# AlphaMistral/Mistral-Water

Measured on AMD Instinct MI355X. Metric: ocean grid-points/sec (full spectrum→IFFT→disp→Jacobian), 1024² grid, 1/2/4/8 GPUs, higher is better.
Workload: dtype f32

## Files before the change

### mistral-water_amd/csrc/ocean_renderer_device.h

```cpp
#pragma once
#include <hip/hip_runtime.h>

#include <mutex>
#include <utility>
#include <vector>

#include "../../include/mistral_water.h"
#include "mw_host.h"
#include "ocean_renderer_kernels.h"
#include "mw_switches.h"

namespace mw {

struct OrTex {
    float* height = nullptr;
    cf* disp = nullptr;
    float *disp_g = nullptr, *normal = nullptr, *white = nullptr;
    float *height_g = nullptr, *disp_a = nullptr;
    OrTex at(size_t texels) const {
        auto mv = [texels](auto* p, size_t per) { return p ? p + per * texels : p; };
        return OrTex{mv(height, 1), mv(disp, 1), mv(disp_g, 1), mv(normal, 3), mv(white, 1), mv(height_g, 1), mv(disp_a, 1)};
    }
    OrTex real_only() const { OrTex t = *this; t.height_g = t.disp_a = nullptr; return t; }
};
// ... 64 lines not shown
#ifndef MW_OR_PACKED_MAX_M
#define MW_OR_PACKED_MAX_M 4096
#endif
#ifndef MW_OR_PACKED
#define MW_OR_PACKED 1
#endif

template <int N, int P>
__global__ __launch_bounds__((OrP1Geom<N, P>::NTHREADS)) void k_or_pass1_packed(OrP1Args A) {
    extern __shared__ __attribute__((aligned(16))) unsigned char smem[];
    using G = OrP1Geom<N, P>;
    cf* lds = reinterpret_cast<cf*>(smem);
    constexpr int T = FftGeom<N, P>::T;
    const int tid = threadIdx.x, jb = blockIdx.x;
    const int f0 = gridDim.y == 1 ? 0 : (int)blockIdx.y, f1 = gridDim.y == 1 ? 2 : f0 + 1;
    {
        const size_t toff = (size_t)blockIdx.z * N * N;
        A.initT += toff; A.PQT += toff; A.phase_in += toff; A.phase_out += toff; A.E += 2 * toff;
    }
    const int w = tid / T, u = tid % T;
    TwStage<N, P, G::NTHREADS, false> tws;
    tws.load(A.TW, tid);
    const Twiddles tw = TwGeom<N, P>::view(A.TW, lds);
    cf* set0 = lds + G::TW_LDS;
    cf h[P], hh[P], x[P];
#pragma unroll
    for (int q = 0; q < P; q++) h[q] = hh[q] = mk(0.f, 0.f);
    if (gridDim.y == 1) or_p1_animate_packed<N, P, MW_OR_P1_CHUNK>(A, jb, tid, true, true, true, h, hh);
    else or_p1_animate_packed<N, P, MW_OR_P1_LONE_CHUNK>(A, jb, tid, f0 == 0, f0 == 0, f0 == 1, h, hh);
    tws.store(lds, tid);
    for (int f = f0; f < f1; f++) {
        or_p1_build_packed<N, P>(A, jb, tid, f, h, hh, x);
        if (f != f0) __syncthreads();
        stage0_store<N, P, -1>(x, u, set0 + w * G::BUFSTRIDE);
        __syncthreads();
#pragma unroll
        for (int s = 1; s < FftGeom<N, P>::S; s++) {
            load_slots<N, P>(x, u, set0 + w * G::BUFSTRIDE, s - 1);
            __syncthreads();
            stage_store<N, P, -1, false>(x, u, set0 + w * G::BUFSTRIDE, tw, s);
            __syncthreads();
        }
        or_p1_finish<N, P>(A, tw, jb, tid, f, x, set0);
    }
}

template <int N, int P>
__global__ __launch_bounds__((OrP1Geom<N, P>::NTHREADS)) void k_or_pass1(OrP1Args A) {
    extern __shared__ __attribute__((aligned(16))) unsigned char smem[];
    using G = OrP1Geom<N, P>;
    cf* lds = reinterpret_cast<cf*>(smem);
    constexpr int T = FftGeom<N, P>::T;
    const int tid = threadIdx.x, jb = blockIdx.x;
    const int f0 = gridDim.y == 1 ? 0 : (int)blockIdx.y, f1 = gridDim.y == 1 ? 3 : f0 + 1;
    {
        const size_t toff = (size_t)blockIdx.z * N * N;
        A.initT += toff; A.phase_in += toff; A.phase_out += toff; A.E += 3 * toff;
    }
    const int w = tid / T, u = tid % T;
    TwStage<N, P, G::NTHREADS, false> tws;
    tws.load(A.TW, tid);
    const Twiddles tw = TwGeom<N, P>::view(A.TW, lds);
    cf* set0 = lds + G::TW_LDS;
    cf h[P], x[P];
    if (gridDim.y == 1) or_p1_animate<N, P, MW_OR_P1_CHUNK>(A, jb, tid, f0 == 0, h);
    else or_p1_animate<N, P, 1>(A, jb, tid, f0 == 0, h);
    tws.store(lds, tid);
    for (int f = f0; f < f1; f++) {
        or_p1_build<N, P>(A, jb, tid, f, h, x);
        if (f != f0) __syncthreads();
        stage0_store<N, P, -1>(x, u, set0 + w * G::BUFSTRIDE);
        __syncthreads();
#pragma unroll
        for (int s = 1; s < FftGeom<N, P>::S; s++) {
            load_slots<N, P>(x, u, set0 + w * G::BUFSTRIDE, s - 1);
            __syncthreads();
            stage_store<N, P, -1, false>(x, u, set0 + w * G::BUFSTRIDE, tw, s);
            __syncthreads();
        }
        or_p1_finish<N, P>(A, tw, jb, tid, f, x, set0);
    }
}

template <int N, int P, bool KEEP, bool PACKED = false>
__global__ __launch_bounds__((OrP1Geom<N, P>::NTHREADS)) void k_or_pass1_steps(OrP1StepsArgs S) {
    constexpr int NF = PACKED ? 2 : 3;
    extern __shared__ __attribute__((aligned(16))) unsigned char smem[];
    using G = OrP1Geom<N, P>;
    cf* lds = reinterpret_cast<cf*>(smem);
    constexpr int T = FftGeom<N, P>::T;
    const int tid = threadIdx.x, jb = blockIdx.x;
    const int k0 = (int)blockIdx.z * S.group, k1 = (k0 + S.group < S.nframes) ? k0 + S.group : S.nframes;
    OrP1Args A = S.a;
    const int w = tid / T, u = tid % T;
    TwStage<N, P, G::NTHREADS, false> tws;
    tws.load(A.TW, tid);
    const Twiddles tw = TwGeom<N, P>::view(A.TW, lds);
    cf* set0 = lds + G::TW_LDS;
    float om[P], ph[P];
    f4 v[P], vn;
    const int fsel = PACKED ? (int)blockIdx.y : 0;
    or_p1_steps_begin<N, P>(A, jb, tid, om, ph);
    float gain[PACKED ? P : 1];
    if constexpr (PACKED) {
        if (KEEP) or_p1_steps_coeff<N, P>(A, jb, tid, fsel, v, vn);
        or_p1_steps_gain<N, P>(A, jb, tid, fsel, gain);
    }
    else { if (KEEP) or_p1_steps_spectrum<N, P>(A, jb, tid, v); }
    tws.store(lds, tid);
    for (int k = 0; k < k0; k++) or_p1_steps_advance<P>(om, ph, S.dt[k]);
    A.E += (size_t)NF * N * N * k0;
    for (int k = k0; k < k1; k++) {
        cf h[PACKED ? 1 : P], x[P];
        or_p1_steps_advance<P>(om, ph, S.dt[k]);
        if constexpr (PACKED) {
            if (!KEEP) or_p1_steps_coeff<N, P>(A, jb, tid, fsel, v, vn);
        } else {
            if (!KEEP) or_p1_steps_spectrum<N, P>(A, jb, tid, v);
            or_p1_steps_animate<P>(v, ph, h);
        }
        for (int f = PACKED ? fsel : 0; f < (PACKED ? fsel + 1 : 3); f++) {
            if constexpr (PACKED) or_p1_steps_build_split<N, P>(tid, f, gain, v, vn, ph, x);
            else or_p1_build<N, P>(A, jb, tid, f, h, x);
            if ((!PACKED && f != 0) || k != k0) __syncthreads();
            stage0_store<N, P, -1>(x, u, set0 + w * G::BUFSTRIDE);
            __syncthreads();
#pragma unroll
            for (int s = 1; s < FftGeom<N, P>::S; s++) {
                load_slots<N, P>(x, u, set0 + w * G::BUFSTRIDE, s - 1);
                __syncthreads();
                stage_store<N, P, -1, false>(x, u, set0 + w * G::BUFSTRIDE, tw, s);
                __syncthreads();
            }
            or_p1_finish<N, P>(A, tw, jb, tid, f, x, set0);
        }
        A.E += (size_t)NF * N * N;
    }
    if (k1 == S.nframes && fsel == 0) or_p1_steps_store_phase<N, P>(A, jb, tid, ph);
}

__global__ __launch_bounds__(256) void k_or_copy_frame(size_t MM, const float* h, const cf* d, const float* dg, const float* n, const float* w,
                                                       const float* hg, const float* da, float* oh, cf* od, float* odg, float* on, float* ow,
                                                       float* ohg, float* oda) {
    const size_t i = (size_t)blockIdx.x * blockDim.x + threadIdx.x, q = MM / 4;
    auto cp = [i](const void* src, void* dst) { reinterpret_cast<f4*>(dst)[i] = reinterpret_cast<const f4*>(src)[i]; };
    if (i < 3 * q) cp(n, on);
    if (i < 2 * q) cp(d, od);
    if (i < q) {
        cp(h, oh); cp(dg, odg); cp(w, ow);
        if (hg) { cp(hg, ohg); cp(da, oda); }
    }
}

__device__ __forceinline__ unsigned or_xcd_band(unsigned b, unsigned nb) { return (nb % 8 == 0) ? (b % 8) * (nb / 8) + b / 8 : b; }
template <int N, int P>
__global__ __launch_bounds__((OrP2Geom<N, P>::NTHREADS)) void k_or_pass2(OrP2Args A) {
    extern __shared__ __attribute__((aligned(16))) unsigned char smem[];
    using G = OrP2Geom<N, P>;
    cf* lds = reinterpret_cast<cf*>(smem);
    constexpr int T = FftGeom<N, P>::T;
    const int tid = threadIdx.x, ab = blockIdx.x;
    {
        const size_t toff = (size_t)blockIdx.z * N * N;
        A.E += 3 * toff; A.height += toff; A.disp += toff; A.disp_g += toff;
        if (A.height_g) A.height_g += toff;
        if (A.disp_a) A.disp_a += toff;
    }
    TwStage<N, P, G::NTHREADS, false> tws;
    tws.load(A.TW, tid);
    const Twiddles tw = TwGeom<N, P>::view(A.TW, lds);
    cf* set0 = lds + G::TW_LDS;
    cf x[P];
    float dx[P];
    const int k0 = blockIdx.y == 0 ? 0 : 2, k1 = blockIdx.y == 0 ? 2 : 3;
    for (int k = k0; k < k1; k++) {
        const int f = or_p2_field(k);
        if (k != k0) __syncthreads();
        or_p2_load<N, P>(A, ab, tid, f, x, set0);
        if (k == k0) tws.store(lds, tid);
        __syncthreads();
#pragma unroll
        for (int s = 1; s < FftGeom<N, P>::S; s++) {
            const int um = XLay<N, P>::EXACT ? tid % FftGeom<N, P>::T : tid >> 2, rm = XLay<N, P>::EXACT ? tid / FftGeom<N, P>::T : tid & 3;
            load_slots<N, P>(x, um, set0 + rm * G::BUFSTRIDE, s - 1);
            __syncthreads();
            stage_store<N, P, -1, false>(x, um, set0 + rm * G::BUFSTRIDE, tw, s);
            __syncthreads();
        }
        or_p2_finish<N, P>(A, tw, ab, tid, f, x, dx, set0);
    }
}

template <int N, int P>
__global__ __launch_bounds__((OrP2Geom<N, P>::NTHREADS)) void k_or_pass2_packed(OrP2Args A) {
    extern __shared__ __attribute__((aligned(16))) unsigned char smem[];
    using G = OrP2Geom<N, P>;
    cf* lds = reinterpret_cast<cf*>(smem);
    const int tid = threadIdx.x, ab = blockIdx.x;
    {
        const size_t toff = (size_t)blockIdx.z * N * N;
        A.E += 2 * toff; A.height += toff; A.disp += toff; A.disp_g += toff;
    }
    TwStage<N, P, G::NTHREADS, false> tws;
    tws.load(A.TW, tid);
    const Twiddles tw = TwGeom<N, P>::view(A.TW, lds);
    cf* set0 = lds + G::TW_LDS;
    cf x[P];
    float dx[P];
    const bool split = gridDim.y == 2;
    const int k0 = split ? (int)blockIdx.y : 0, k1 = split ? k0 + 1 : 2;
    for (int k = k0; k < k1; k++) {
        if (k != k0) __syncthreads();
        or_p2_load<N, P>(A, ab, tid, k, x, set0);
        if (k == k0) tws.store(lds, tid);
        __syncthreads();
#pragma unroll
        for (int s = 1; s < FftGeom<N, P>::S; s++) {
            const int um = XLay<N, P>::EXACT ? tid % FftGeom<N, P>::T : tid >> 2, rm = XLay<N, P>::EXACT ? tid / FftGeom<N, P>::T : tid & 3;
            load_slots<N, P>(x, um, set0 + rm * G::BUFSTRIDE, s - 1);
            __syncthreads();
            stage_store<N, P, -1, false>(x, um, set0 + rm * G::BUFSTRIDE, tw, s);
// ... 152 lines not shown
    return A;
}
template <int N>
static hipError_t or_launch_passes(OrState& s, float dt, bool imag, hipStream_t st, hipEvent_t* ev = nullptr) {
    constexpr int P = Plan<N>::P;
    static AttrOnce attr1, attr2;
    hipError_t e = attr1.set(reinterpret_cast<const void*>(&k_or_pass1<N, P>), OrP1Geom<N, P>::LDS_BYTES);
    if (e == hipSuccess) e = attr2.set(reinterpret_cast<const void*>(&k_or_pass2<N, P>), OrP2Geom<N, P>::LDS_BYTES);
    if (e != hipSuccess) return e;
    const OrP1Args A1 = or_p1_args(s, s.initT, s.PQT, s.phaseT2, s.E, dt, or_call_is_big(s));
    const OrP2Args A2 = or_p2_args(s, s.E, imag ? s.out : s.out.real_only());
    constexpr int NT1 = OrP1Geom<N, P>::NTHREADS, LB1 = OrP1Geom<N, P>::LDS_BYTES;
    constexpr int NT2 = OrP2Geom<N, P>::NTHREADS, LB2 = OrP2Geom<N, P>::LDS_BYTES;
    const bool packed = or_use_packed(s, imag), all_fields = or_all_fields(s);
    if constexpr (N < MW_OR_PACKED_MAX_M) if (packed) {
        static AttrOnce attr1p, attr2p;
        e = attr1p.set(reinterpret_cast<const void*>(&k_or_pass1_packed<N, P>), LB1);
        if (e == hipSuccess) e = attr2p.set(reinterpret_cast<const void*>(&k_or_pass2_packed<N, P>), LB2);
        if (e != hipSuccess) return e;
        if (ev) hipEventRecord(ev[0], st);
        k_or_pass1_packed<N, P><<<dim3(N / 4, all_fields ? 1 : 2, s.tiles), dim3(NT1), LB1, st>>>(A1);
        if (ev) hipEventRecord(ev[1], st);
        std::swap(s.phaseT, s.phaseT2);
        k_or_pass2_packed<N, P><<<dim3(N / 4, all_fields ? 1 : 2, s.tiles), dim3(NT2), LB2, st>>>(A2);
        if (ev) hipEventRecord(ev[2], st);
        return hipGetLastError();
    }
    if (ev) hipEventRecord(ev[0], st);
    k_or_pass1<N, P><<<dim3(N / 4, all_fields ? 1 : 3, s.tiles), dim3(NT1), LB1, st>>>(A1);
    if (ev) hipEventRecord(ev[1], st);
    std::swap(s.phaseT, s.phaseT2);
    k_or_pass2<N, P><<<dim3(N / 4, 2, s.tiles), dim3(NT2), LB2, st>>>(A2);
    if (ev) hipEventRecord(ev[2], st);
    return hipGetLastError();
}

static inline mw_status or_generate(OrState& s, float delta_time, bool imag, float* d_height, float* d_disp, float* d_normal, float* d_white,
                                    hipStream_t st, hipEvent_t* ev = nullptr) {
    const float dt = delta_time * s.mult;
    const mw_status r = imag ? or_imag_planes(s) : MW_OK;
    if (r != MW_OK) return r;
    hipError_t e = hipSuccess;
    MW_FOR_SIZE(s.M, return fail(MW_EINVAL, "OceanRenderer: unsupported texture size"), e = or_launch_passes<NN>(s, dt, imag, st, ev));
    if (e != hipSuccess) return fail(MW_EDEVICE, std::string("OceanRenderer pass launch: ") + hipGetErrorString(e));
    const size_t MM = (size_t)s.M * s.M, TM = MM * (size_t)s.tiles;
    const unsigned nb = or_nw_blocks(MM);
    const OrTex& o = s.out;
    if (or_call_is_big(s)) k_or_normal_white<true><<<dim3(nb, s.tiles), dim3(256), 0, st>>>(s.c, o.height, o.disp, o.disp_g, o.normal, o.white);
    else k_or_normal_white<false><<<dim3(nb, s.tiles), dim3(256), 0, st>>>(s.c, o.height, o.disp, o.disp_g, o.normal, o.white);
    if (hipGetLastError() != hipSuccess) return fail(MW_EDEVICE, "OceanRenderer normal/white launch failed");
    if (ev) hipEventRecord(ev[3], st);
    s.have_frame = true;
    hipError_t ce = hipSuccess;
    if (d_height && ce == hipSuccess) ce = hipMemcpyAsync(d_height, o.height, TM * 4, hipMemcpyDeviceToDevice, st);
    if (d_disp && ce == hipSuccess) ce = hipMemcpyAsync(d_disp, o.disp, TM * 8, hipMemcpyDeviceToDevice, st);
    if (d_normal && ce == hipSuccess) ce = hipMemcpyAsync(d_normal, o.normal, TM * 12, hipMemcpyDeviceToDevice, st);
    if (d_white && ce == hipSuccess) ce = hipMemcpyAsync(d_white, o.white, TM * 4, hipMemcpyDeviceToDevice, st);
    if (ce != hipSuccess) return fail(MW_EDEVICE, std::string("OceanRenderer result copy: ") + hipGetErrorString(ce));
    if (ev) hipEventRecord(ev[4], st);
    return MW_OK;
}

static inline mw_status or_frames_reserve(OrState& s, int n, const bool (&need)[4], bool imag) {
    if (n > s.frames_cap) {
        or_release(s, OR_B_FRAMES);
        s.frames_cap = 0; s.frames_last = 0;
    }
    const size_t cap = (size_t)(s.frames_cap ? s.frames_cap : n);
    const unsigned when = OR_B_FR | (need[0] ? OR_B_FR_HEIGHT : 0u) | (need[1] ? OR_B_FR_DISP : 0u) | (need[2] ? OR_B_FR_NORMAL : 0u) |
                          (need[3] ? OR_B_FR_WHITE : 0u) | (imag ? OR_B_FR_IMAG : 0u);
    if (!or_alloc(s, when, 0, cap)) {
        (void)hipGetLastError();
        return fail(MW_ENOMEM, "OceanRenderer: hipMalloc of the frame buffers failed");
    }
    s.frames_cap = (int)cap;
    return MW_OK;
}
#ifndef MW_OR_FRAME_GROUPS
#define MW_OR_FRAME_GROUPS 4
#endif
#ifndef MW_OR_FRAME_GROUPS_PACKED
#define MW_OR_FRAME_GROUPS_PACKED 2
#endif
#ifndef MW_OR_STEPS_CHUNK
#define MW_OR_STEPS_CHUNK 8
#endif
static inline int or_steps_chunk(int M) {
    const long long c = (long long)MW_OR_STEPS_CHUNK * 1024 * 1024 / ((long long)M * M);
    return c < 1 ? 1 : (c > MW_OR_MAX_FRAMES ? MW_OR_MAX_FRAMES : (int)c);
}
static inline int or_steps_chunks(int M, int n) { const int c = or_steps_chunk(M); return (n + c - 1) / c; }
#ifndef MW_OR_STEPS_MAX_N
#define MW_OR_STEPS_MAX_N 2048
#endif
template <int N, bool PACKED>
static hipError_t or_launch_steps(OrState& s, const float* dt, int n, const OrTex& f, hipStream_t st, hipEvent_t* ev = nullptr) {
    constexpr int P = Plan<N>::P, NF = PACKED ? 2 : 3;
    constexpr bool KEEP = P <= 8;
    static AttrOnce attr1, attr2;
    {
        hipError_t e;
        if constexpr (PACKED) e = attr2.set(reinterpret_cast<const void*>(&k_or_pass2_packed<N, P>), OrP2Geom<N, P>::LDS_BYTES);
        else e = attr2.set(reinterpret_cast<const void*>(&k_or_pass2<N, P>), OrP2Geom<N, P>::LDS_BYTES);
        if (e != hipSuccess) return e;
    }
    constexpr int NT1 = OrP1Geom<N, P>::NTHREADS, LB1 = OrP1Geom<N, P>::LDS_BYTES;
    if (ev) hipEventRecord(ev[0], st);
    constexpr int NT2 = OrP2Geom<N, P>::NTHREADS, LB2 = OrP2Geom<N, P>::LDS_BYTES;
    const size_t MM = (size_t)N * N;
    const int chunk = or_steps_chunk(N);
    auto rest = [&](int c0, int cn, int j) {
        const OrTex c = f.at(MM * (size_t)c0);
        const OrP2Args B2 = or_p2_args(s, s.fr_E + NF * MM * (size_t)c0, c);
        if constexpr (PACKED) k_or_pass2_packed<N, P><<<dim3(N / 4, 1, cn), dim3(NT2), LB2, st>>>(B2);
        else k_or_pass2<N, P><<<dim3(N / 4, 2, cn), dim3(NT2), LB2, st>>>(B2);
        if (ev) hipEventRecord(ev[2 + 3 * j], st);
        k_or_normal_white<true><<<dim3(or_nw_blocks(MM), cn), dim3(256), 0, st>>>(s.c, c.height, c.disp, c.disp_g, c.normal, c.white);
        if (ev) hipEventRecord(ev[3 + 3 * j], st);
    };
    if constexpr (N <= MW_OR_STEPS_MAX_N) {
        hipError_t e = attr1.set(reinterpret_cast<const void*>(&k_or_pass1_steps<N, P, KEEP, PACKED>), LB1);
        if (e != hipSuccess) return e;
        OrP1StepsArgs S;
        S.a = or_p1_args(s, s.initT, s.PQT, s.phaseT2, s.fr_E, 0.f, true);
        for (int k = 0; k < MW_OR_MAX_FRAMES; k++) S.dt[k] = k < n ? dt[k] : 0.f;
        S.nframes = n;
        int groups = PACKED ? MW_OR_FRAME_GROUPS_PACKED : MW_OR_FRAME_GROUPS;
        if (groups > n) groups = n;
        S.group = (n + groups - 1) / groups;
        groups = (n + S.group - 1) / S.group;
        k_or_pass1_steps<N, P, KEEP, PACKED><<<dim3(N / 4, PACKED ? 2 : 1, groups), dim3(NT1), LB1, st>>>(S);
        for (int c0 = 0, j = 0; c0 < n; c0 += chunk, j++) {
            if (ev) hipEventRecord(ev[1 + 3 * j], st);
            rest(c0, (n - c0 < chunk) ? n - c0 : chunk, j);
        }
        std::swap(s.phaseT, s.phaseT2);
    } else {
        hipError_t e;
        if constexpr (PACKED) e = attr1.set(reinterpret_cast<const void*>(&k_or_pass1_packed<N, P>), LB1);
        else e = attr1.set(reinterpret_cast<const void*>(&k_or_pass1<N, P>), LB1);
        if (e != hipSuccess) return e;
        for (int c0 = 0, j = 0; c0 < n; c0 += chunk, j++) {
            const int cn = (n - c0 < chunk) ? n - c0 : chunk;
            for (int k = c0; k < c0 + cn; k++) {
                const OrP1Args A1 = or_p1_args(s, s.initT, s.PQT, s.phaseT2, s.fr_E + (size_t)NF * N * N * k, dt[k], true);
                if constexpr (PACKED) k_or_pass1_packed<N, P><<<dim3(N / 4, 1, 1), dim3(NT1), LB1, st>>>(A1);
                else k_or_pass1<N, P><<<dim3(N / 4, 1, 1), dim3(NT1), LB1, st>>>(A1);
                std::swap(s.phaseT, s.phaseT2);
            }
            if (ev) hipEventRecord(ev[1 + 3 * j], st);
            rest(c0, cn, j);
        }
    }
    return hipGetLastError();
}
static inline mw_status or_generate_steps(OrState& s, const float* delta_time, int n, bool imag, float* d_height, float* d_disp, float* d_normal,
                                          float* d_white, hipStream_t st, hipEvent_t* ev = nullptr) {
    if (s.tiles != 1) return fail(MW_ESTATE, "generate_texture_steps: a batched handle (mw_ocean_create_batch) advances one frame per call");
    if (n < 1 || n > MW_OR_MAX_FRAMES) return fail(MW_EINVAL, "generate_texture_steps: nframes out of range");
    const size_t MM = (size_t)s.M * s.M;
    mw_status r = imag ? or_imag_planes(s) : MW_OK;
    if (r != MW_OK) return r;
    const bool need[4] = {!d_height, !d_disp, !d_normal, !d_white};
    if ((r = or_frames_reserve(s, n, need, imag)) != MW_OK) return r;
    float dt[MW_OR_MAX_FRAMES];
    for (int k = 0; k < n; k++) dt[k] = delta_time[k] * s.mult;
    OrTex f = imag ? s.fr : s.fr.real_only();
    if (d_height) f.height = d_height;
    if (d_disp) f.disp = reinterpret_cast<cf*>(d_disp);
    if (d_normal) f.normal = d_normal;
    if (d_white) f.white = d_white;
    hipError_t e = hipSuccess;
    const bool packed = or_use_packed(s, imag);
    MW_FOR_SIZE(s.M, return fail(MW_EINVAL, "OceanRenderer: unsupported texture size"),
                e = packed ? or_launch_steps<NN, (NN < MW_OR_PACKED_MAX_M)>(s, dt, n, f, st, ev) : or_launch_steps<NN, false>(s, dt, n, f, st, ev));
    if (e != hipSuccess) return fail(MW_EDEVICE, std::string("OceanRenderer steps launch: ") + hipGetErrorString(e));
    const OrTex l = f.at((size_t)(n - 1) * MM), &o = s.out;
    k_or_copy_frame<<<dim3((unsigned)((3 * MM / 4 + 255) / 256)), dim3(256), 0, st>>>(MM, l.height, l.disp, l.disp_g, l.normal, l.white, l.height_g, l.disp_a,
                                                                                     o.height, o.disp, o.disp_g, o.normal, o.white, o.height_g, o.disp_a);
    if (hipGetLastError() != hipSuccess) return fail(MW_EDEVICE, "OceanRenderer normal/white launch failed");
    if (ev) hipEventRecord(ev[1 + 3 * or_steps_chunks(s.M, n)], st);
    s.have_frame = true;
    return MW_OK;
}

static inline mw_status or_frames(OrState& s, float choppiness, const float* delta_time, int n, bool rgba, void* const (&d)[4], hipStream_t st,
                                  hipEvent_t* ev = nullptr) {
    s.c.choppiness = choppiness;
    float* const p[4] = {rgba ? nullptr : (float*)d[0], rgba ? nullptr : (float*)d[1], rgba ? nullptr : (float*)d[2], rgba ? nullptr : (float*)d[3]};
    const mw_status r = n == 1 ? or_generate(s, delta_time[0], rgba, p[0], p[1], p[2], p[3], st, ev)
                               : or_generate_steps(s, delta_time, n, rgba, p[0], p[1], p[2], p[3], st, ev);
    if (r != MW_OK || !rgba) return r;
    const size_t MM = (size_t)s.M * s.M;
    const OrTex& t = n == 1 ? s.out : s.fr;
    k_or_pack_rgba<<<dim3((unsigned)((MM + 255) / 256), n == 1 ? s.tiles : n), dim3(256), 0, st>>>(s.M, t.height, t.height_g, t.disp, t.disp_g, t.disp_a, t.normal,
                                                                                              t.white, (f4*)d[0], (f4*)d[1], (f4*)d[2], (f4*)d[3]);
    if (hipGetLastError() != hipSuccess) return fail(MW_EDEVICE, "k_or_pack_rgba launch failed");
    return MW_OK;
}

struct OrAdvanceArgs {
    float dt[MW_OR_MAX_FRAMES];
    int n;
};
__global__ __launch_bounds__(256) void k_or_advance(size_t MM, const float* omT, float* phase, OrAdvanceArgs A) {
    const size_t i = (size_t)blockIdx.x * blockDim.x + threadIdx.x;
    if (i >= MM) return;
    const float om = omT[i];
    float ph = phase[i + (size_t)blockIdx.y * MM];
    for (int k = 0; k < A.n; k++) ph = or_phase_step(om, ph, A.dt[k]);
    phase[i + (size_t)blockIdx.y * MM] = ph;
}
static inline mw_status or_advance_phase(OrState& s, const float* delta_time, int n, hipStream_t st) {
    const size_t MM = (size_t)s.M * s.M;
// ... 23 lines not shown
```

### mistral-water_amd/csrc/ocean_renderer_kernels.h

```cpp
#pragma once
#include "fftmesh_kernels.h"

namespace mw {

struct OrConsts {
    int M;
    float length, gravity, choppiness;
    float normal_length;
};

MW_HD float or_wave(int M, float length, int p) {
    const float n = (float)((p < M / 2) ? p : p - M);
    return sdiv(smul(smul(2.0f, MW_PI_F), n), length);
}
MW_HD float or_phillips(int M, float length, float wind_x, float wind_y, float amp, float gravity, float kx, float kz) {
    float klen = sqrtf(kx * kx + kz * kz);
    float klen2 = klen * klen, klen4 = klen2 * klen2;
    if (klen < MW_EPS_F) return 0.f;
    float wlen = sqrtf(wind_x * wind_x + wind_y * wind_y);
    float kDotW = (kx / klen) * (wind_x / wlen) + (kz / klen) * (wind_y / wlen);
    float l = wlen * wlen / gravity, l2 = l * l;
    float damping = 0.01f, L2 = l2 * damping * damping;
    return amp * expf(-1.f / (klen2 * l2)) / klen4 * (kDotW * kDotW) * expf(-klen2 * L2);
}
// ... 17 lines not shown
    }
    f4 v;
    v.x = o[0]; v.y = o[1]; v.z = o[2]; v.w = -o[3];
    initT[(size_t)px * M + py] = v;
    if (phaseT) phaseT[(size_t)px * M + py] = 0.f;
}
MW_HD float or_omega(const OrConsts& c, int px, int py) {
    const float kx = or_wave(c.M, c.length, px), kz = or_wave(c.M, c.length, py);
    const float wlen = ssqrt(sadd(smul(kx, kx), smul(kz, kz)));
    const float q = sdiv(sdiv(smul(wlen, wlen), 370.f), 370.f);
    const float inner = smul(smul(c.gravity, wlen), sadd(1.f, q));
    return ssqrt(inner);
}
MW_HD float or_phase_step(float omega, float old_phase, float dt) {
    const float x = sadd(old_phase, smul(omega, dt)), twopi = smul(2.0f, MW_PI_F);
    if (x >= 0.f && x < twopi) return x;
    if (x >= twopi && x < sadd(twopi, twopi)) return ssub(x, twopi);
    return fmodf(x, twopi);
}
MW_HD float or_phase_advance(const OrConsts& c, int px, int py, float old_phase, float dt) {
    return or_phase_step(or_omega(c, px, py), old_phase, dt);
}

struct OrP1Args {
    const f4* PQT;
    const f4* initT;
    const float* omT;
    const float* phase_in;
    float* phase_out;
    const cf* TW;
    cf* E;
    OrConsts c;
    float dt;
    int stream_E;
};
template <int N, int P>
struct OrP1Geom {
    static constexpr int T = FftGeom<N, P>::T;
    static constexpr int NTHREADS = 4 * T;
    static constexpr int BUFSTRIDE = FftGeom<N, P>::LBUF + (XLay<N, P>::EXACT ? XLay<N, P>::PAD_RD4 : 4);
    static constexpr int TW_LDS = (TwGeom<N, P>::LDS_CF + 1) & ~1;
    static constexpr int LDS_BYTES = (TW_LDS + 4 * BUFSTRIDE) * (int)sizeof(cf);
};
#ifndef MW_OR_P1_CHUNK
#define MW_OR_P1_CHUNK 8
#endif
template <int N, int P, int CH_>
MW_HD void or_p1_animate(const OrP1Args& A, int jb, int tid, bool write_phase, cf (&h)[P]) {
    constexpr int T = FftGeom<N, P>::T;
    const int w = wave_uniform<(T % 64) == 0>(tid / T), u = tid % T, px = 4 * jb + w;
    const size_t col = (size_t)px * N;
    const float* const c_om = A.omT + col;
    const float* const c_pi = A.phase_in + col;
    float* const c_po = A.phase_out + col;
    const f4* const c_in = A.initT + col;
    const unsigned uo = (unsigned)u;
    constexpr int CH = P < CH_ ? P : CH_;
#pragma unroll
    for (int q0 = 0; q0 < P; q0 += CH) {
        float om[CH], pi[CH];
        f4 v[CH];
#pragma unroll
        for (int k = 0; k < CH; k++) {
            om[k] = (c_om + T * (q0 + k))[uo];
            pi[k] = (c_pi + T * (q0 + k))[uo];
            v[k] = (c_in + T * (q0 + k))[uo];
        }
#pragma unroll
        for (int k = 0; k < CH; k++) {
            const float ph = or_phase_step(om[k], pi[k], A.dt);
            if (write_phase) (c_po + T * (q0 + k))[uo] = ph;
            float s, c;
            mw_sincos(ph, &s, &c);
            h[q0 + k] = animate(v[k].x, v[k].y, v[k].z, v[k].w, c, s);
        }
    }
}
#define MW_OR_MAX_FRAMES 32
struct OrP1StepsArgs {
    OrP1Args a;
    float dt[MW_OR_MAX_FRAMES];
    int nframes, group;
};
template <int N, int P>
MW_HD void or_p1_steps_begin(const OrP1Args& A, int jb, int tid, float (&om)[P], float (&ph)[P]) {
    constexpr int T = FftGeom<N, P>::T;
    const int w = wave_uniform<(T % 64) == 0>(tid / T), u = tid % T, px = 4 * jb + w;
    const size_t col = (size_t)px * N;
    const float* const c_om = A.omT + col;
    const float* const c_pi = A.phase_in + col;
    const unsigned uo = (unsigned)u;
#pragma unroll
    for (int q = 0; q < P; q++) {
        om[q] = (c_om + T * q)[uo];
        ph[q] = (c_pi + T * q)[uo];
    }
}
template <int N, int P>
MW_HD void or_p1_steps_spectrum(const OrP1Args& A, int jb, int tid, f4 (&v)[P]) {
    constexpr int T = FftGeom<N, P>::T;
    const int w = wave_uniform<(T % 64) == 0>(tid / T), u = tid % T, px = 4 * jb + w;
    const f4* const c_in = A.initT + (size_t)px * N;
    const unsigned uo = (unsigned)u;
#pragma unroll
    for (int q = 0; q < P; q++) v[q] = (c_in + T * q)[uo];
}
template <int P>
MW_HD void or_p1_steps_advance(const float (&om)[P], float (&ph)[P], float dt) {
#pragma unroll
    for (int q = 0; q < P; q++) ph[q] = or_phase_step(om[q], ph[q], dt);
}
template <int P>
MW_HD void or_p1_steps_animate(const f4 (&v)[P], const float (&ph)[P], cf (&h)[P]) {
#pragma unroll
    for (int q = 0; q < P; q++) {
        float s, c;
        mw_sincos(ph[q], &s, &c);
        h[q] = animate(v[q].x, v[q].y, v[q].z, v[q].w, c, s);
    }
}
template <int N, int P>
MW_HD void or_p1_steps_store_phase(const OrP1Args& A, int jb, int tid, const float (&ph)[P]) {
    constexpr int T = FftGeom<N, P>::T;
    const int w = wave_uniform<(T % 64) == 0>(tid / T), u = tid % T, px = 4 * jb + w;
    float* const c_po = A.phase_out + (size_t)px * N;
    const unsigned uo = (unsigned)u;
#pragma unroll
    for (int q = 0; q < P; q++) (c_po + T * q)[uo] = ph[q];
}

MW_HD float or_gain(float kc, float kx, float kz, float chop) {
    const float wl = fmaxf(0.0001f, sqrtf(__builtin_fmaf(kx, kx, smul(kz, kz))));
    return smul(sdiv(kc, wl), chop);
}
template <int N, int P>
MW_HD void or_p1_build(const OrP1Args& A, int jb, int tid, int f, const cf (&h)[P], cf (&x)[P]) {
    constexpr int T = FftGeom<N, P>::T;
    const int w = tid / T, u = tid % T, px = 4 * jb + w;
    const float kx = or_wave(N, A.c.length, px);
#pragma unroll
    for (int q = 0; q < P; q++) {
        if (f == 0) { x[q] = h[q]; continue; }
        const float kz = or_wave(N, A.c.length, u + T * q);
        const float g = or_gain((f == 1) ? kx : kz, kx, kz, A.c.choppiness);
        x[q] = mk(smul(h[q].y, g), smul(-h[q].x, g));
    }
}
MW_HD void or_prep_element(int M, int px, int py, const f4* initT, f4* PQT) {
    const int mx = (M - px) % M, my = (M - py) % M;
    const f4 a = initT[(size_t)px * M + py], b = initT[(size_t)mx * M + my];
    f4 o;
    o.x = smul(0.5f, sadd(a.x, b.z)); o.y = smul(0.5f, ssub(a.y, b.w));
    o.z = smul(0.5f, sadd(a.z, b.x)); o.w = smul(0.5f, ssub(a.w, b.y));
    PQT[(size_t)px * M + py] = o;
}
template <int N, int P>
MW_HD void or_p1_build_packed(const OrP1Args& A, int jb, int tid, int f, const cf (&h)[P], const cf (&hh)[P], cf (&x)[P]) {
    constexpr int T = FftGeom<N, P>::T;
    const int w = tid / T, u = tid % T, px = 4 * jb + w;
    const float kx = or_wave(N, A.c.length, px);
#pragma unroll
    for (int q = 0; q < P; q++) {
        const int py = u + T * q;
        const float kz = or_wave(N, A.c.length, py);
        const float g = or_gain((f == 0) ? kx : kz, kx, kz, A.c.choppiness);
        if (f == 0) { x[q] = mk(smul(h[q].y, g), smul(-h[q].x, g)); continue; }
        const bool nyq = (py == N / 2);
        const float tx = nyq ? ssub(h[q].x, hh[q].x) : hh[q].x, ty = nyq ? ssub(h[q].y, hh[q].y) : hh[q].y;
        x[q] = mk(sadd(hh[q].x, smul(g, tx)), sadd(hh[q].y, smul(g, ty)));
    }
}
template <int N, int P, int CH_>
MW_HD void or_p1_animate_packed(const OrP1Args& A, int jb, int tid, bool write_phase, bool want_h, bool want_hh, cf (&h)[P], cf (&hh)[P]) {
    constexpr int T = FftGeom<N, P>::T;
    const int w = wave_uniform<(T % 64) == 0>(tid / T), u = tid % T, px = 4 * jb + w;
    const size_t col = (size_t)px * N;
    const float* const c_om = A.omT + col;
    const float* const c_pi = A.phase_in + col;
    float* const c_po = A.phase_out + col;
    const f4* const c_in = A.initT + col;
    const f4* const c_pq = A.PQT + col;
    const unsigned uo = (unsigned)u;
    constexpr int CH = P < CH_ ? P : CH_;
#pragma unroll
    for (int q0 = 0; q0 < P; q0 += CH) {
        float om[CH], pi[CH];
        f4 v[CH], pq[CH];
#pragma unroll
        for (int k = 0; k < CH; k++) {
            om[k] = (c_om + T * (q0 + k))[uo];
            pi[k] = (c_pi + T * (q0 + k))[uo];
            if (want_h || (q0 + k) == P / 2) v[k] = (c_in + T * (q0 + k))[uo];
            if (want_hh) pq[k] = (c_pq + T * (q0 + k))[uo];
        }
#pragma unroll
        for (int k = 0; k < CH; k++) {
            const float ph = or_phase_step(om[k], pi[k], A.dt);
            if (write_phase) (c_po + T * (q0 + k))[uo] = ph;
            float s, c;
            mw_sincos(ph, &s, &c);
            if (want_h || (q0 + k) == P / 2) h[q0 + k] = animate(v[k].x, v[k].y, v[k].z, v[k].w, c, s);
            if (want_hh) hh[q0 + k] = animate(pq[k].x, pq[k].y, pq[k].z, pq[k].w, c, s);
        }
    }
}
template <int N, int P>
MW_HD void or_p1_steps_coeff(const OrP1Args& A, int jb, int tid, int f, f4 (&c)[P], f4& vn) {
    constexpr int T = FftGeom<N, P>::T;
    const int w = wave_uniform<(T % 64) == 0>(tid / T), u = tid % T, px = 4 * jb + w;
    const f4* const c_c = (f == 0 ? A.initT : A.PQT) + (size_t)px * N;
    const unsigned uo = (unsigned)u;
#pragma unroll
    for (int q = 0; q < P; q++) c[q] = (c_c + T * q)[uo];
    vn = (A.initT + (size_t)px * N + T * (P / 2))[uo];
}
template <int N, int P>
MW_HD void or_p1_steps_gain(const OrP1Args& A, int jb, int tid, int f, float (&g)[P]) {
    constexpr int T = FftGeom<N, P>::T;
    const int w = tid / T, u = tid % T, px = 4 * jb + w;
    const float kx = or_wave(N, A.c.length, px);
#pragma unroll
    for (int q = 0; q < P; q++) {
        const float kz = or_wave(N, A.c.length, u + T * q);
        g[q] = or_gain((f == 0) ? kx : kz, kx, kz, A.c.choppiness);
    }
}
template <int N, int P>
MW_HD void or_p1_steps_build_split(int tid, int f, const float (&g_)[P], const f4 (&c)[P], const f4& vn, const float (&ph)[P], cf (&x)[P]) {
    constexpr int T = FftGeom<N, P>::T;
    const int u = tid % T;
#pragma unroll
    for (int q = 0; q < P; q++) {
        float sn, cs;
        mw_sincos(ph[q], &sn, &cs);
        const cf a = animate(c[q].x, c[q].y, c[q].z, c[q].w, cs, sn);
        const int py = u + T * q;
        const float g = g_[q];
        if (f == 0) { x[q] = mk(smul(a.y, g), smul(-a.x, g)); continue; }
        float tx = a.x, ty = a.y;
        if (q == P / 2) {
            const cf hn = animate(vn.x, vn.y, vn.z, vn.w, cs, sn);
            const bool nyq = (py == N / 2);
            tx = nyq ? ssub(hn.x, a.x) : a.x;
            ty = nyq ? ssub(hn.y, a.y) : a.y;
        }
        x[q] = mk(sadd(a.x, smul(g, tx)), sadd(a.y, smul(g, ty)));
    }
}

template <int N, int P>
MW_HD void or_p1_finish(const OrP1Args& A, const Twiddles& tw, int jb, int tid, int f, cf (&x)[P], const cf* lds) {
    constexpr int T = FftGeom<N, P>::T;
    const int w2 = tid & 3, u2 = tid >> 2;
    load_last<N, P>(x, u2, lds + w2 * OrP1Geom<N, P>::BUFSTRIDE);
    final_stage<N, P, -1>(x, u2, tw.TF);
    cf* Ef = A.E + (size_t)f * N * N + (size_t)jb * N * 4;
    const unsigned to = (unsigned)tid;
    if (A.stream_E) {
#pragma unroll
        for (int q = 0; q < P; q++) mw_store_stream<true>(&(Ef + (size_t)4 * T * q)[to], x[q]);
    } else {
#pragma unroll
        for (int q = 0; q < P; q++) (Ef + (size_t)4 * T * q)[to] = x[q];
    }
}

struct OrP2Args {
    const cf* E;
    const cf* TW;
    float* height;
    cf* disp;
    float* disp_g;
    float* height_g;
    float* disp_a;
    OrConsts c;
};
template <int N, int P>
struct OrP2Geom {
    static constexpr int T = FftGeom<N, P>::T;
    static constexpr int R2 = 4;
    static constexpr int NTHREADS = R2 * T;
    static constexpr int BUFSTRIDE = FftGeom<N, P>::LBUF + (XLay<N, P>::EXACT ? XLay<N, P>::PAD_WR4 : 4);
    static constexpr int TW_LDS = (TwGeom<N, P>::LDS_CF + 1) & ~1;
    static constexpr int LDS_BYTES = (TW_LDS + R2 * BUFSTRIDE) * (int)sizeof(cf);
};
MW_HD int or_p2_field(int k) { return k == 0 ? 1 : (k == 1 ? 2 : 0); }
template <int N, int P>
MW_HD void or_p2_load(const OrP2Args& A, int ab, int tid, int f, cf (&x)[P], cf* lds) {
    constexpr int T = FftGeom<N, P>::T;
    const int r1 = tid & 3, u1 = tid >> 2, row = ab * 4 + r1;
    const cf* Ef = A.E + (size_t)f * N * N;
#pragma unroll
    for (int q = 0; q < P; q++) {
        const int j = u1 + T * q;
        x[q] = Ef[((size_t)(j >> 2) * N + row) * 4 + (j & 3)];
    }
    stage0_store<N, P, -1>(x, u1, lds + r1 * OrP2Geom<N, P>::BUFSTRIDE);
}
template <int N, int P>
MW_HD void or_p2_finish(const OrP2Args& A, const Twiddles& tw, int ab, int tid, int f, cf (&x)[P], float (&dx)[P],
                        const cf* lds) {
    constexpr int T = FftGeom<N, P>::T;
    const int g = wave_uniform<(T % 64) == 0>(tid / T), u = tid % T, a = ab * 4 + g;
    load_last<N, P>(x, u, lds + g * OrP2Geom<N, P>::BUFSTRIDE);
    final_stage<N, P, -1>(x, u, tw.TF);
    const size_t rowoff = (size_t)a * N;
    float* const r_dg = A.disp_g + rowoff;
    cf* const r_d = A.disp + rowoff;
    float* const r_da = A.disp_a ? A.disp_a + rowoff : nullptr;
    float* const r_h = A.height + rowoff;
    float* const r_hg = A.height_g ? A.height_g + rowoff : nullptr;
    const unsigned uo = (unsigned)u;
#pragma unroll
    for (int q = 0; q < P; q++) {
        if (f == 1) { dx[q] = x[q].x; (r_dg + T * q)[uo] = x[q].y; }
        else if (f == 2) { (r_d + T * q)[uo] = mk(dx[q], x[q].x); if (r_da) (r_da + T * q)[uo] = x[q].y; }
        else if (f == 3) { (r_d + T * q)[uo] = mk(dx[q], x[q].y); (r_h + T * q)[uo] = x[q].x; }
        else if (f == 4) { (reinterpret_cast<float*>(r_d) + 2 * T * q)[2 * uo] = x[q].x; (r_dg + T * q)[uo] = x[q].y; }
        else if (f == 5) { (reinterpret_cast<float*>(r_d) + 2 * T * q)[2 * uo + 1] = x[q].y; (r_h + T * q)[uo] = x[q].x; }
        else { (r_h + T * q)[uo] = x[q].x; if (r_hg) (r_hg + T * q)[uo] = x[q].y; }
    }
}

MW_HD int or_clamp(int v, int hi) { return v < 0 ? 0 : (v > hi ? hi : v); }
MW_HD void or_normal_math(float ts, float cx, float cy, float cz, float rx, float rh, float rz, float lx, float lh, float lz, float tx,
                          float th, float tz, float bx, float bh, float bz, float (&n)[3]) {
    const float r0 = ts + rx - cx, r1 = rh - cy, r2 = rz - cz;
    const float l0 = -ts + lx - cx, l1 = lh - cy, l2 = lz - cz;
    const float t0 = tx - cx, t1 = th - cy, t2 = -ts + tz - cz;
    const float b0 = bx - cx, b1 = bh - cy, b2 = ts + bz - cz;
    float nx = (r1 * t2 - r2 * t1) + (t1 * l2 - t2 * l1) + (l1 * b2 - l2 * b1) + (b1 * r2 - b2 * r1);
// ... 135 lines not shown
```

Measured before the change: 82.56 billion.

## Fuse the two packed field workgroups into one and share sincos through LDS

Adds a DUO variant of the pass-1 steps kernel. It merges the two packed-field workgroups into a single double-width workgroup. Each half advances phases and computes sincos for only half of the slots, then exchanges the results through a shared LDS area. This removes the duplicated phase loads, phase advance and sincos work that both field workgroups used to repeat. The trade-offs are a larger workgroup, more LDS per block, fewer blocks (frame groups default to 1 for this path), and an extra barrier per frame, all of which could lower occupancy and parallelism.

```diff
diff --git a/mistral-water_amd/csrc/ocean_renderer_device.h b/mistral-water_amd/csrc/ocean_renderer_device.h
--- a/mistral-water_amd/csrc/ocean_renderer_device.h
+++ b/mistral-water_amd/csrc/ocean_renderer_device.h
@@ -170,47 +170,61 @@
     }
 }
 
-template <int N, int P, bool KEEP, bool PACKED = false>
-__global__ __launch_bounds__((OrP1Geom<N, P>::NTHREADS)) void k_or_pass1_steps(OrP1StepsArgs S) {
+template <int N, int P, bool KEEP, bool PACKED = false, bool DUO = false>
+__global__ __launch_bounds__(((DUO ? 2 : 1) * OrP1Geom<N, P>::NTHREADS)) void k_or_pass1_steps(OrP1StepsArgs S) {
+    static_assert(!DUO || (PACKED && KEEP && OrP1Duo<N, P>::value), "the two-field workgroup is a form of the packed plan with the coefficients kept");
     constexpr int NF = PACKED ? 2 : 3;
     extern __shared__ __attribute__((aligned(16))) unsigned char smem[];
     using G = OrP1Geom<N, P>;
     cf* lds = reinterpret_cast<cf*>(smem);
-    constexpr int T = FftGeom<N, P>::T;
-    const int tid = threadIdx.x, jb = blockIdx.x;
+    constexpr int T = FftGeom<N, P>::T, NT = G::NTHREADS;
+    constexpr int PC = DUO ? P / 2 : P;
+    const int half = DUO ? wave_uniform<(NT % 64) == 0>((int)threadIdx.x / NT) : 0;
+    const int tid = DUO ? (int)threadIdx.x - half * NT : (int)threadIdx.x, jb = blockIdx.x;
     const int k0 = (int)blockIdx.z * S.group, k1 = (k0 + S.group < S.nframes) ? k0 + S.group : S.nframes;
     OrP1Args A = S.a;
     const int w = tid / T, u = tid % T;
-    TwStage<N, P, G::NTHREADS, false> tws;
-    tws.load(A.TW, tid);
+    TwStage<N, P, (DUO ? 2 : 1) * NT, false> tws;
+    tws.load(A.TW, threadIdx.x);
     const Twiddles tw = TwGeom<N, P>::view(A.TW, lds);
-    cf* set0 = lds + G::TW_LDS;
-    float om[P], ph[P];
+    const int fsel = DUO ? half : (PACKED ? (int)blockIdx.y : 0);
+    cf* set0 = lds + G::TW_LDS + (DUO ? half * 4 * G::BUFSTRIDE : 0);
+    const int q0 = DUO ? half * PC : 0;
+    float om[PC], ph[PC];
     f4 v[P], vn;
-    const int fsel = PACKED ? (int)blockIdx.y : 0;
-    or_p1_steps_begin<N, P>(A, jb, tid, om, ph);
+    or_p1_steps_begin<N, P, PC>(A, jb, tid, q0, om, ph);
     float gain[PACKED ? P : 1];
     if constexpr (PACKED) {
         if (KEEP) or_p1_steps_coeff<N, P>(A, jb, tid, fsel, v, vn);
         or_p1_steps_gain<N, P>(A, jb, tid, fsel, gain);
     }
     else { if (KEEP) or_p1_steps_spectrum<N, P>(A, jb, tid, v); }
-    tws.store(lds, tid);
-    for (int k = 0; k < k0; k++) or_p1_steps_advance<P>(om, ph, S.dt[k]);
+    tws.store(lds, threadIdx.x);
+    for (int k = 0; k < k0; k++) or_p1_steps_advance<PC>(om, ph, S.dt[k]);
     A.E += (size_t)NF * N * N * k0;
     for (int k = k0; k < k1; k++) {
-        cf h[PACKED ? 1 : P], x[P];
-        or_p1_steps_advance<P>(om, ph, S.dt[k]);
-        if constexpr (PACKED) {
+        cf h[PACKED ? 1 : P], x[P], sc[DUO ? P : 1];
+        or_p1_steps_advance<PC>(om, ph, S.dt[k]);
+        if constexpr (DUO) {
+            cf* xs = lds + OrP1Duo<N, P>::XS;
+            cf own[PC];
+            or_p1_steps_sincos<PC>(ph, own);
+#pragma unroll
+            for (int q = 0; q < PC; q++) xs[(q0 + q) * NT + tid] = own[q];
+            __syncthreads();
+#pragma unroll
+            for (int q = 0; q < P; q++) sc[q] = xs[q * NT + tid];
+        } else if constexpr (PACKED) {
             if (!KEEP) or_p1_steps_coeff<N, P>(A, jb, tid, fsel, v, vn);
         } else {
             if (!KEEP) or_p1_steps_spectrum<N, P>(A, jb, tid, v);
             or_p1_steps_animate<P>(v, ph, h);
         }
         for (int f = PACKED ? fsel : 0; f < (PACKED ? fsel + 1 : 3); f++) {
-            if constexpr (PACKED) or_p1_steps_build_split<N, P>(tid, f, gain, v, vn, ph, x);
+            if constexpr (DUO) or_p1_steps_build_field<N, P>(tid, f, gain, v, vn, sc, x);
+            else if constexpr (PACKED) or_p1_steps_build_split<N, P>(tid, f, gain, v, vn, ph, x);
             else or_p1_build<N, P>(A, jb, tid, f, h, x);
-            if ((!PACKED && f != 0) || k != k0) __syncthreads();
+            if (!DUO && ((!PACKED && f != 0) || k != k0)) __syncthreads();
             stage0_store<N, P, -1>(x, u, set0 + w * G::BUFSTRIDE);
             __syncthreads();
 #pragma unroll
@@ -224,7 +238,7 @@
         }
         A.E += (size_t)NF * N * N;
     }
-    if (k1 == S.nframes && fsel == 0) or_p1_steps_store_phase<N, P>(A, jb, tid, ph);
+    if (k1 == S.nframes && (DUO || fsel == 0)) or_p1_steps_store_phase<N, P, PC>(A, jb, tid, q0, ph);
 }
 
 __global__ __launch_bounds__(256) void k_or_copy_frame(size_t MM, const float* h, const cf* d, const float* dg, const float* n, const float* w,
@@ -543,6 +557,9 @@
 #ifndef MW_OR_FRAME_GROUPS_PACKED
 #define MW_OR_FRAME_GROUPS_PACKED 2
 #endif
+#ifndef MW_OR_FRAME_GROUPS_DUO
+#define MW_OR_FRAME_GROUPS_DUO 1
+#endif
 #ifndef MW_OR_STEPS_CHUNK
 #define MW_OR_STEPS_CHUNK 8
 #endif
@@ -580,17 +597,19 @@
         if (ev) hipEventRecord(ev[3 + 3 * j], st);
     };
     if constexpr (N <= MW_OR_STEPS_MAX_N) {
-        hipError_t e = attr1.set(reinterpret_cast<const void*>(&k_or_pass1_steps<N, P, KEEP, PACKED>), LB1);
+        constexpr bool DUO = PACKED && KEEP && OrP1Duo<N, P>::value;
+        constexpr int NTS = DUO ? OrP1Duo<N, P>::NTHREADS : NT1, LBS = DUO ? OrP1Duo<N, P>::LDS_BYTES : LB1;
+        hipError_t e = attr1.set(reinterpret_cast<const void*>(&k_or_pass1_steps<N, P, KEEP, PACKED, DUO>), LBS);
         if (e != hipSuccess) return e;
         OrP1StepsArgs S;
         S.a = or_p1_args(s, s.initT, s.PQT, s.phaseT2, s.fr_E, 0.f, true);
         for (int k = 0; k < MW_OR_MAX_FRAMES; k++) S.dt[k] = k < n ? dt[k] : 0.f;
         S.nframes = n;
-        int groups = PACKED ? MW_OR_FRAME_GROUPS_PACKED : MW_OR_FRAME_GROUPS;
+        int groups = DUO ? MW_OR_FRAME_GROUPS_DUO : (PACKED ? MW_OR_FRAME_GROUPS_PACKED : MW_OR_FRAME_GROUPS);
         if (groups > n) groups = n;
         S.group = (n + groups - 1) / groups;
         groups = (n + S.group - 1) / S.group;
-        k_or_pass1_steps<N, P, KEEP, PACKED><<<dim3(N / 4, PACKED ? 2 : 1, groups), dim3(NT1), LB1, st>>>(S);
+        k_or_pass1_steps<N, P, KEEP, PACKED, DUO><<<dim3(N / 4, (PACKED && !DUO) ? 2 : 1, groups), dim3(NTS), LBS, st>>>(S);
         for (int c0 = 0, j = 0; c0 < n; c0 += chunk, j++) {
             if (ev) hipEventRecord(ev[1 + 3 * j], st);
             rest(c0, (n - c0 < chunk) ? n - c0 : chunk, j);
diff --git a/mistral-water_amd/csrc/ocean_renderer_kernels.h b/mistral-water_amd/csrc/ocean_renderer_kernels.h
--- a/mistral-water_amd/csrc/ocean_renderer_kernels.h
+++ b/mistral-water_amd/csrc/ocean_renderer_kernels.h
@@ -123,16 +123,16 @@
     float dt[MW_OR_MAX_FRAMES];
     int nframes, group;
 };
-template <int N, int P>
-MW_HD void or_p1_steps_begin(const OrP1Args& A, int jb, int tid, float (&om)[P], float (&ph)[P]) {
+template <int N, int P, int PC>
+MW_HD void or_p1_steps_begin(const OrP1Args& A, int jb, int tid, int q0, float (&om)[PC], float (&ph)[PC]) {
     constexpr int T = FftGeom<N, P>::T;
     const int w = wave_uniform<(T % 64) == 0>(tid / T), u = tid % T, px = 4 * jb + w;
     const size_t col = (size_t)px * N;
-    const float* const c_om = A.omT + col;
-    const float* const c_pi = A.phase_in + col;
-    const unsigned uo = (unsigned)u;
-#pragma unroll
-    for (int q = 0; q < P; q++) {
+    const float* const c_om = A.omT + col + T * q0;
+    const float* const c_pi = A.phase_in + col + T * q0;
+    const unsigned uo = (unsigned)u;
+#pragma unroll
+    for (int q = 0; q < PC; q++) {
         om[q] = (c_om + T * q)[uo];
         ph[q] = (c_pi + T * q)[uo];
     }
@@ -146,10 +146,10 @@
 #pragma unroll
     for (int q = 0; q < P; q++) v[q] = (c_in + T * q)[uo];
 }
-template <int P>
-MW_HD void or_p1_steps_advance(const float (&om)[P], float (&ph)[P], float dt) {
-#pragma unroll
-    for (int q = 0; q < P; q++) ph[q] = or_phase_step(om[q], ph[q], dt);
+template <int PC>
+MW_HD void or_p1_steps_advance(const float (&om)[PC], float (&ph)[PC], float dt) {
+#pragma unroll
+    for (int q = 0; q < PC; q++) ph[q] = or_phase_step(om[q], ph[q], dt);
 }
 template <int P>
 MW_HD void or_p1_steps_animate(const f4 (&v)[P], const float (&ph)[P], cf (&h)[P]) {
@@ -160,14 +160,14 @@
         h[q] = animate(v[q].x, v[q].y, v[q].z, v[q].w, c, s);
     }
 }
-template <int N, int P>
-MW_HD void or_p1_steps_store_phase(const OrP1Args& A, int jb, int tid, const float (&ph)[P]) {
+template <int N, int P, int PC>
+MW_HD void or_p1_steps_store_phase(const OrP1Args& A, int jb, int tid, int q0, const float (&ph)[PC]) {
     constexpr int T = FftGeom<N, P>::T;
     const int w = wave_uniform<(T % 64) == 0>(tid / T), u = tid % T, px = 4 * jb + w;
-    float* const c_po = A.phase_out + (size_t)px * N;
-    const unsigned uo = (unsigned)u;
-#pragma unroll
-    for (int q = 0; q < P; q++) (c_po + T * q)[uo] = ph[q];
+    float* const c_po = A.phase_out + (size_t)px * N + T * q0;
+    const unsigned uo = (unsigned)u;
+#pragma unroll
+    for (int q = 0; q < PC; q++) (c_po + T * q)[uo] = ph[q];
 }
 
 MW_HD float or_gain(float kc, float kx, float kz, float chop) {
@@ -266,28 +266,56 @@
         g[q] = or_gain((f == 0) ? kx : kz, kx, kz, A.c.choppiness);
     }
 }
-template <int N, int P>
-MW_HD void or_p1_steps_build_split(int tid, int f, const float (&g_)[P], const f4 (&c)[P], const f4& vn, const float (&ph)[P], cf (&x)[P]) {
-    constexpr int T = FftGeom<N, P>::T;
-    const int u = tid % T;
-#pragma unroll
-    for (int q = 0; q < P; q++) {
+template <int PC>
+MW_HD void or_p1_steps_sincos(const float (&ph)[PC], cf (&sc)[PC]) {
+#pragma unroll
+    for (int q = 0; q < PC; q++) {
         float sn, cs;
         mw_sincos(ph[q], &sn, &cs);
-        const cf a = animate(c[q].x, c[q].y, c[q].z, c[q].w, cs, sn);
-        const int py = u + T * q;
-        const float g = g_[q];
-        if (f == 0) { x[q] = mk(smul(a.y, g), smul(-a.x, g)); continue; }
-        float tx = a.x, ty = a.y;
-        if (q == P / 2) {
-            const cf hn = animate(vn.x, vn.y, vn.z, vn.w, cs, sn);
-            const bool nyq = (py == N / 2);
-            tx = nyq ? ssub(hn.x, a.x) : a.x;
-            ty = nyq ? ssub(hn.y, a.y) : a.y;
-        }
-        x[q] = mk(sadd(a.x, smul(g, tx)), sadd(a.y, smul(g, ty)));
-    }
-}
+        sc[q] = mk(sn, cs);
+    }
+}
+template <int N, int P>
+MW_HD cf or_p1_steps_build_point(int u, int q, int f, float g, const f4& c, const f4& vn, float sn, float cs) {
+    constexpr int T = FftGeom<N, P>::T;
+    const cf a = animate(c.x, c.y, c.z, c.w, cs, sn);
+    if (f == 0) return mk(smul(a.y, g), smul(-a.x, g));
+    float tx = a.x, ty = a.y;
+    if (q == P / 2) {
+        const cf hn = animate(vn.x, vn.y, vn.z, vn.w, cs, sn);
+        const bool nyq = (u + T * q == N / 2);
+        tx = nyq ? ssub(hn.x, a.x) : a.x;
+        ty = nyq ? ssub(hn.y, a.y) : a.y;
+    }
+    return mk(sadd(a.x, smul(g, tx)), sadd(a.y, smul(g, ty)));
+}
+template <int N, int P>
+MW_HD void or_p1_steps_build_field(int tid, int f, const float (&g)[P], const f4 (&c)[P], const f4& vn, const cf (&sc)[P], cf (&x)[P]) {
+    const int u = tid % FftGeom<N, P>::T;
+#pragma unroll
+    for (int q = 0; q < P; q++) x[q] = or_p1_steps_build_point<N, P>(u, q, f, g[q], c[q], vn, sc[q].x, sc[q].y);
+}
+template <int N, int P>
+MW_HD void or_p1_steps_build_split(int tid, int f, const float (&g)[P], const f4 (&c)[P], const f4& vn, const float (&ph)[P], cf (&x)[P]) {
+    const int u = tid % FftGeom<N, P>::T;
+#pragma unroll
+    for (int q = 0; q < P; q++) {
+        float sn, cs;
+        mw_sincos(ph[q], &sn, &cs);
+        x[q] = or_p1_steps_build_point<N, P>(u, q, f, g[q], c[q], vn, sn, cs);
+    }
+}
+#ifndef MW_OR_DUO_MIN_N
+#define MW_OR_DUO_MIN_N 1024
+#endif
+template <int N, int P>
+struct OrP1Duo {
+    using G = OrP1Geom<N, P>;
+    static constexpr bool value = N >= MW_OR_DUO_MIN_N && P <= 8 && P % 2 == 0 && 2 * G::NTHREADS <= 1024;
+    static constexpr int NTHREADS = 2 * G::NTHREADS;
+    static constexpr int XS = G::TW_LDS + 8 * G::BUFSTRIDE;
+    static constexpr int LDS_BYTES = (XS + P * G::NTHREADS) * (int)sizeof(cf);
+};
 
 template <int N, int P>
 MW_HD void or_p1_finish(const OrP1Args& A, const Twiddles& tw, int jb, int tid, int f, cf (&x)[P], const cf* lds) {
```

After: 82.86 billion (median of 3 runs). No clear change (+0.4%).
